# AnishDelft/ModelCompression

Measured on AMD Instinct MI355X. Metric: images/sec (fwd+bwd, 416x416), higher is better.
Workload: dtype fp16

## Files before the change

include/mcamd.h:

```cpp
#ifndef MCAMD_H
#define MCAMD_H

#include <stddef.h>
#include <stdint.h>

#ifdef __cplusplus
extern "C" {
#endif

#define MCAMD_OK 0
#define MCAMD_EINVAL (-1)
#define MCAMD_ELAUNCH (-2)
#define MCAMD_EWORKSPACE (-3)

int mcamd_version(void);
void mcamd_reload_config(void);
const char* mcamd_arch(void);
const char* mcamd_last_error(void);

typedef struct mcamd_conv_geom {
    int32_t B, H, W;
    int32_t ksize;
    int32_t cin;
    int32_t cout;
// ... 164 lines not shown
    int32_t ch_lo, C;
} mcamd_dgrad_sums;
int32_t mcamd_conv_dgrad_sums_rows(const mcamd_conv_geom* g, int32_t concurrent);
int mcamd_conv_dgrad_sums(const mcamd_conv_geom* g, const void* dy, int32_t dy_ld, int32_t dy_choff,
                          const void* wp_dgrad, const mcamd_conv_epilogue* epi, const mcamd_dgrad_sums* sums, void* stream);

size_t mcamd_conv_wgrad_workspace_bytes(const mcamd_conv_geom* g);
int mcamd_conv_wgrad(const mcamd_conv_geom* g, const void* x, const void* dy, int32_t dy_ld,
                     int32_t dy_choff, const float* mask_oihw, const mcamd_chan_map* map,
                     float grad_scale, float* dw_oihw, float* dbias, void* workspace,
                     size_t workspace_bytes, void* stream);

#define MCAMD_WGRAD_GENERIC 0
#define MCAMD_WGRAD_STEM 1
#define MCAMD_WGRAD_WIN 2
#define MCAMD_WGRAD_NINE 3
#define MCAMD_WGRAD_NINE_WIDE 4
#define MCAMD_WFIN_ROW 0
#define MCAMD_WFIN_VEC 1
#define MCAMD_WFIN_GENERIC 2
#define MCAMD_WGRAD_PLAN_INFO_N 13
int mcamd_conv_wgrad_plan_info(const mcamd_conv_geom* g, int32_t has_cmap, int32_t out[MCAMD_WGRAD_PLAN_INFO_N]);
int32_t mcamd_wgrad_generic_instances(int32_t* out, int32_t cap);

int mcamd_bn_coeffs(const float* stats, int32_t stats_rows, int32_t stats_ld, int32_t C, int64_t count,
                    const float* gamma, const float* beta, float* running_mean, float* running_var,
                    float momentum, float eps, int32_t training,
                    float* scale, float* shift, float* save_mean, float* save_invstd,
                    const int32_t* chan_perm, void* stream);

int mcamd_bn_coeffs_ex(const float* stats, int32_t stats_rows, int32_t stats_ld, int32_t C, int64_t count,
                       const float* gamma, const float* beta, float* running_mean, float* running_var,
                       float momentum, float eps, int32_t training,
                       float* scale, float* shift, float* save_mean, float* save_invstd,
                       const int32_t* chan_perm, int32_t ones_channel, void* stream);

#define MCAMD_DST_PLAIN 0
#define MCAMD_DST_POOL 1
#define MCAMD_DST_REORG 2
typedef struct mcamd_act_desc {
    int32_t B, H, W, C;
    const void* y; int32_t y_ld, y_choff;
    const float* scale; const float* shift;
    float slope;
    int32_t mode;
    void* dst; int32_t dst_ld, dst_choff;
// ... 353 lines not shown
```

modelcompression_amd/_lib.py:

```python
import ctypes as C
import os

_HERE = os.path.dirname(os.path.abspath(__file__))
LIB_PATH = os.path.join(_HERE, "libmcamd.so")


class McamdError(RuntimeError):
    pass


class ConvGeom(C.Structure):
    _fields_ = [("B", C.c_int32), ("H", C.c_int32), ("W", C.c_int32), ("ksize", C.c_int32),
                ("cin", C.c_int32), ("cout", C.c_int32), ("x_ld", C.c_int32), ("x_choff", C.c_int32),
                ("stem", C.c_int32), ("pad", C.c_int32), ("x_wrap", C.c_int32), ("x_f8", C.c_int32), ("x_f8_wexp", C.c_int32)]


class ConvEpilogue(C.Structure):
    _fields_ = [("mode", C.c_int32), ("y_ld", C.c_int32), ("y_choff", C.c_int32),
                ("y", C.c_void_p), ("bias", C.c_void_p), ("stats", C.c_void_p),
                ("stats_rows", C.c_int32), ("stats_ld", C.c_int32),
                ("scale", C.c_void_p), ("shift", C.c_void_p), ("slope", C.c_float), ("overflow", C.c_void_p),
                ("dst_mode", C.c_int32), ("y2", C.c_void_p), ("y2_ld", C.c_int32), ("y2_choff", C.c_int32),
                ("concurrent", C.c_int32)]

# ... 215 lines not shown
    "mcamd_conv_fwd_q8_sparse24_ok": (_I32, [C.POINTER(ConvGeom)]),
    "mcamd_q8_sparse24_elems": (C.c_int, [C.POINTER(ConvGeom), C.POINTER(_I64)]),
    "mcamd_pack_q8_sparse24": (C.c_int, [C.POINTER(ConvGeom), _P, _P, _P, _P, _P, _P]),
    "mcamd_conv_fwd_q8_sparse24": (C.c_int, [C.POINTER(ConvGeom), _P, _P, _P, _P, C.POINTER(ConvEpilogue), _I32, _I32, _P]),
    "mcamd_conv_fwd_q8_w4_ok": (_I32, [C.POINTER(ConvGeom)]),
    "mcamd_q8_w4_elems": (C.c_int, [C.POINTER(ConvGeom), C.POINTER(_I64)]),
    "mcamd_pack_q8_w4": (C.c_int, [C.POINTER(ConvGeom), _P, _P, _P, _P, _P, _P]),
    "mcamd_unpack_q8_w4": (C.c_int, [C.POINTER(ConvGeom), _P, _P, _P, _P]),
    "mcamd_conv_fwd_q8_w4": (C.c_int, [C.POINTER(ConvGeom), _P, _P, _P, _P, C.POINTER(ConvEpilogue), _I32, _I32, _P]),
    "mcamd_conv_fwd_q8_w4_info": (C.c_int, [C.POINTER(ConvGeom), C.POINTER(_I32)]),
    "mcamd_conv_fwd_q8_w4_raw": (C.c_int, [C.POINTER(ConvGeom), _P, _P, _P, _P, C.POINTER(ConvEpilogue), _P]),
    "mcamd_fakequant_q8_w4": (C.c_int, [C.POINTER(ConvGeom), _P, _P, _P, _P, _P]),
    "mcamd_cast_q8": (C.c_int, [_P, _I64, _I32, _I32, _I32, _P, _I32, _I32, _P]),
    "mcamd_conv_fwd_q8_stats_rows": (_I32, [C.POINTER(ConvGeom)]),
    "mcamd_fakequant_q8": (C.c_int, [C.POINTER(ConvGeom), _P, _P, _P, _P, _P]),
    "mcamd_cast_q8_train": (C.c_int, [_P, _I64, _I32, _I32, _I32, _P, _I32, _I32, _P]),
    "mcamd_conv_dgrad": (C.c_int, [C.POINTER(ConvGeom), _P, _I32, _I32, _P, C.POINTER(ConvEpilogue), _P]),
    "mcamd_conv_dgrad_sums_rows": (_I32, [C.POINTER(ConvGeom), _I32]),
    "mcamd_conv_dgrad_sums": (C.c_int, [C.POINTER(ConvGeom), _P, _I32, _I32, _P, C.POINTER(ConvEpilogue), C.POINTER(DgradSums), _P]),
    "mcamd_conv_wgrad_workspace_bytes": (_SZ, [C.POINTER(ConvGeom)]),
    "mcamd_conv_wgrad": (C.c_int, [C.POINTER(ConvGeom), _P, _P, _I32, _I32, _P, C.POINTER(ChanMap), _F, _P, _P, _P, _SZ, _P]),
    "mcamd_conv_wgrad_plan_info": (C.c_int, [C.POINTER(ConvGeom), _I32, C.POINTER(_I32)]),
    "mcamd_wgrad_generic_instances": (_I32, [C.POINTER(_I32), _I32]),
    "mcamd_bn_coeffs": (C.c_int, [_P, _I32, _I32, _I32, _I64, _P, _P, _P, _P, _F, _F, _I32, _P, _P, _P, _P, _P, _P]),
    "mcamd_bn_coeffs_ex": (C.c_int, [_P, _I32, _I32, _I32, _I64, _P, _P, _P, _P, _F, _F, _I32, _P, _P, _P, _P, _P, _I32, _P]),
    "mcamd_fold_weights": (C.c_int, [C.POINTER(FoldDesc), _P, _P]),
    "mcamd_fold_weights_many": (C.c_int, [_P, _I32, _I64, _P]),
    "mcamd_unfold_wgrad": (C.c_int, [C.POINTER(FoldDesc), _P, _P, _P, _P, _I32, _P]),
    "mcamd_bn_act_fwd": (C.c_int, [C.POINTER(ActDesc), _P]),
    "mcamd_bn_act_fwd_instance": (C.c_int, [C.POINTER(ActDesc), C.POINTER(ActInstance)]),
    "mcamd_bn_act_conv1x1_ok": (_I32, [C.POINTER(ActDesc), C.POINTER(ConvGeom)]),
    "mcamd_bn_act_conv1x1_stats_rows": (_I32, [C.POINTER(ActDesc), C.POINTER(ConvGeom)]),
    "mcamd_bn_act_conv1x1_info": (C.c_int, [C.POINTER(ActDesc), C.POINTER(ConvGeom), C.POINTER(BnConv1x1Instance)]),
    "mcamd_bn_act_conv1x1_fwd": (C.c_int, [C.POINTER(ActDesc), C.POINTER(ConvGeom), _P, C.POINTER(ConvEpilogue), _P]),
    "mcamd_bn_act_bwd_workspace_bytes": (_SZ, [C.POINTER(ActBwdDesc)]),
    "mcamd_bn_act_bwd": (C.c_int, [C.POINTER(ActBwdDesc), _P, _SZ, _P]),
    "mcamd_stem_block_workspace_bytes": (_SZ, []),
    "mcamd_stem_block_fwd": (C.c_int, [C.POINTER(StemBlockDesc), _P, _SZ, _P]),
    "mcamd_stem_block_bwd": (C.c_int, [C.POINTER(StemBlockDesc), _P, _SZ, _P]),
    "mcamd_stem_block_stats_rows": (_I32, [C.POINTER(StemBlockDesc)]),
    "mcamd_stem_block_stats": (C.c_int, [C.POINTER(StemBlockDesc), _P, _I32, _I32, _P]),
    "mcamd_stem_block_plan_info": (C.c_int, [C.POINTER(StemBlockDesc), C.POINTER(_I32)]),
    "mcamd_nchw_f32_to_nhwc4_split": (C.c_int, [_P, _I32, _I32, _I32, _P, _P, _P]),
    "mcamd_pack_stem_split": (C.c_int, [_P, _P, _I32, _P, _P, _P]),
    "mcamd_nchw_f32_to_padded_nhwc_f16": (C.c_int, [_P, _I32, _I32, _I32, _I32, _F, _P, _I32, _I32, _P, _P]),
    "mcamd_nchw_f32_to_padded_nhwc_f16_pad": (C.c_int, [_P, _I32, _I32, _I32, _I32, _F, _P, _I32, _I32, _I32, _P, _P]),
# ... 94 lines not shown
```

modelcompression_amd/build.py:

```python
import os
import subprocess
import sys
from concurrent.futures import ThreadPoolExecutor

HERE = os.path.dirname(os.path.abspath(__file__))
CSRC = os.path.join(HERE, "csrc")
OUT = os.path.join(HERE, "libmcamd.so")
HIPCC = os.environ.get("HIPCC", "/opt/rocm/bin/hipcc")
ARCH = "gfx950"
COMMON = ["--offload-arch=" + ARCH, "-O3", "-fPIC", "-std=c++17", "-Wall", "-Wno-unused-variable",
          "-fhip-fp32-correctly-rounded-divide-sqrt"]
SOURCES = {
    "api.hip": [],
    "conv_igemm.hip": [],
    "conv_igemm_pp.hip": [],
    "conv_sparse.hip": [],
    "conv_bsparse.hip": [],
    "conv_splitk.hip": [],
    "conv_q8.hip": [],
    "conv_q8_sparse.hip": [],
    "conv_q8_splitk.hip": [],
    "conv_q8_bsparse.hip": [],
    "conv_q8_w4.hip": [],
    "conv_stem.hip": [],
    "conv_stem_block.hip": [],
    "conv_stem_f32.hip": [],
    "conv_small.hip": [],
    "conv_win.hip": [],
    "conv_wres.hip": [],
    "conv_wgrad.hip": [],
    "conv_wgrad_stem.hip": [],
    "bn_act.hip": [],
    "bn_conv1x1.hip": [],
    "fold.hip": [],
    "plan.hip": [],
    "region_loss.hip": [],
    "distill_loss.hip": [],
    "prune.hip": ["-ffp-contract=off"],
    "augment.hip": ["-ffp-contract=off"],
    "detect.hip": ["-ffp-contract=off"],
    "voc_eval.hip": ["-ffp-contract=off"],
    "wpack.hip": ["-ffp-contract=off"],
    "wshare.hip": ["-ffp-contract=off"],
    "huff.hip": [],
    "taylor.hip": ["-ffp-contract=off"],
}


def _stale(target, deps):
    if not os.path.exists(target):
        return True
    t = os.path.getmtime(target)
    return any(os.path.getmtime(d) > t for d in deps)

# ... 34 lines not shown
```

modelcompression_amd/csrc/api.hip:

```cpp
#include <stdarg.h>
#include <stdlib.h>
#include <string.h>

#include <string>

#include "kernels.h"

static thread_local char g_err[512] = "";

void mcamd_set_error(const char* fmt, ...) {
    va_list ap;
    va_start(ap, fmt);
    vsnprintf(g_err, sizeof(g_err), fmt, ap);
    va_end(ap);
}

int g_mcamd_env_generation = 0;
int McamdEnvSlot::get(const char* name, int dflt) {
    const int g = __atomic_load_n(&g_mcamd_env_generation, __ATOMIC_ACQUIRE);
    if (gen != g) {
        const char* s = getenv(name);
        has = s && *s ? 1 : 0;
        val = has ? atoi(s) : 0;
        __atomic_store_n(&gen, g, __ATOMIC_RELEASE);
// ... 1312 lines not shown
    a.dy_off = dy_choff + a.dy_row_stride + dy_ld;
    a.dy_zero_off = dy_choff;
    a.H = g->H, a.W = g->W, a.HW = g->H * g->W;
    a.M = (int)M;
    a.cin_tap = cin_tap;
    a.ntaps = ntaps;
    a.ktot = ntaps * cin_tap;
    fill_taps(g->ksize, g->stem, a.x_row_stride, g->x_ld, a.tap_off);
    int rc = p.nine    ? mcamd_wgrad9_launch(a, p, g->W + pw_of(g), padded_pixels(g), st)
             : p.stemw == 1 ? mcamd_wgrad_stem_launch(a, p, st)
             : p.stemw == 2 ? mcamd_wgrad_win_launch(a, p, st)
                       : mcamd_wgrad_launch(a, p, st);
    if (rc) return rc;
    rc = mcamd_wgrad_finish_launch((const float*)workspace, p, a.ktot, cin_tap, g->stem, g->cout, g->cin, g->ksize,
                                   mask_oihw, 1.0f / grad_scale, dw_oihw, rmap, cmap, st);
    if (rc) return rc;
    if (dbias) {
        long long rows = padded_pixels(g);
        rc = mcamd_colsum_launch((const half_t*)dy, rows, dy_ld, dy_choff, g->cout, 1.0f / grad_scale, dbias, st, workspace,
                                 workspace_bytes);
    }
    return rc;
}
```

modelcompression_amd/csrc/kernels.h:

```cpp
#pragma once
#include "common.h"

struct DgradSums {
    float* slab;
    const half_t* act;
    const float* scale;
    const float* shift;
    const float* mean;
    const float* invstd;
    const float* y;
    int act_ld, act_choff, act_pw;
    int y_ld, y_choff;
    int ch_lo, C;
    int ld;
    float slope;
};
#define MCAMD_EPI_RAW_F16_SUMS 4

struct IgemmArgs {
    const half_t* x;
    const half_t* w;
    void* y;
    const float* bias;
    float* stats;
// ... 134 lines not shown
int mcamd_conv_q8_w4_raw_launch(IgemmArgs& a, const void* gshift, const void* wexp, hipStream_t st);
int mcamd_fakequant_q8_w4_launch(const void* codes, const void* gshift, const void* wexp, float* out, int cout, int cin, int ntaps,
                                 hipStream_t st);

WgradPlan mcamd_wgrad_plan(long long M, int cout, int cin_tap, int ntaps);
int mcamd_wgrad_launch(WgradArgs& a, const WgradPlan& p, hipStream_t st);
bool mcamd_wgrad_stem_ok(int stem, int cout, int W, long long M);
WgradPlan mcamd_wgrad_stem_plan(long long M);
int mcamd_wgrad_stem_launch(WgradArgs& a, const WgradPlan& p, hipStream_t st);
bool mcamd_wgrad_win_ok(int ksize, int stem, int cout, int cin_tap, int W, long long M);
WgradPlan mcamd_wgrad_win_plan(long long M, int cout);
int mcamd_wgrad_win_launch(WgradArgs& a, const WgradPlan& p, hipStream_t st);
bool mcamd_wgrad_use9(int ksize, int stem, int cout, int cin_tap, int W);
WgradPlan mcamd_wgrad_plan9(long long P, int cout, int cin_tap, int W, int pitch, int B);
int mcamd_wgrad9_launch(const WgradArgs& w, const WgradPlan& p, int pitch, long long P, hipStream_t st);
WgradFinish mcamd_wgrad_finish_pick(int nsplit, int stem, int Cin, int ksize, bool has_cmap);
int mcamd_wgrad_instances(int (*out)[4], int cap);
int mcamd_wgrad_finish_launch(const float* slab, const WgradPlan& p, int ktot, int cin_tap, int stem, int Cout, int Cin,
                              int ksize, const float* mask, float inv_scale, float* dw, const int* rmap, const int* cmap,
                              hipStream_t st);
int mcamd_colsum_launch(const half_t* dy, long long rows, int ld, int choff, int C, float inv_scale, float* out,
                        hipStream_t st, void* scratch, size_t scratch_bytes);

bool mcamd_win3x3_ok(int mode, bool stats, long long M, int n, int cin_tap, int ktot, int H, int W);
int mcamd_win3x3_launch(const IgemmArgs& a, hipStream_t st);
bool mcamd_small3x3_ok(long long M, int n, int cin_tap, int ktot);
int mcamd_small3x3_rows(long long M);
int mcamd_small3x3_launch(const IgemmArgs& a, int rows, hipStream_t st);
bool mcamd_small3x3_split_ok(long long M, int n, int cin_tap, int ktot, int wrap, int mode);
int mcamd_small3x3_split_launch(const IgemmArgs& a, int rows, hipStream_t st);

bool mcamd_bn_conv1x1_shape_ok(int P, int cout);
struct BnConv1x1Choice { int bn, cb, threads, rows, num_mtiles, grid, lds_bytes; };
bool mcamd_bn_conv1x1_choice(int P, int cout, long long M, int rows, BnConv1x1Choice* c);
int mcamd_bn_conv1x1_launch(IgemmArgs& a, const float* py, int py_ld, int py_choff, int P, int rows, hipStream_t st);

bool mcamd_wres_ok(int ksize, int stem, int n, int cin_tap, int ktot, int B, int H, int W, int mode);
int mcamd_wres_rows(int n, int B, int H, int W);
int mcamd_wres_launch(IgemmArgs& a, int B, int rows, hipStream_t st);

bool mcamd_stem_direct_ok(int stem, int cout, int mode);
int mcamd_stem_rows(long long M);
int mcamd_stem_launch(const StemArgs& a, int cout, int rows, hipStream_t st);
```

modelcompression_amd/engine.py:

```python
import contextlib
import math
import os
import time

import torch

from . import ops
from . import _lib as L
from ._lib import McamdError


class _T:
    __slots__ = ("buf", "ld", "choff", "C", "H", "W", "ps", "ps0")

    def __init__(self, buf, ld, choff, C, H, W, ps=0):
        self.buf, self.ld, self.choff, self.C, self.H, self.W, self.ps = buf, ld, choff, C, H, W, ps
        self.ps0 = ps


_LAYER_FIELDS = dict(
    index=0, li=0, conv=None, bn=None, slope=1.0, src=0, tin=None, cin=0, cout=0, cout_p=0, H=0, W=0, k=0, M=0, stem=0, pad=0,
    level=1, mode=0, out_id=None, out2_id=None, out_t=None, out2_t=None, is_last=False, train_ok=True, border=None,
    border_map=None, geom=None, geom_f=None, p_lo=0, p_hi=0,
    wp=None, wd=None, y=None, stats=None, scale=None, shift=None, mean=None, invstd=None, dy=None, gin=None, act_full=None,
# ... 309 lines not shown
        self.overlap_wgrad = os.environ.get("MCAMD_OVERLAP_WGRAD", "1") == "1"
        self.wgrad_chunk = 1
        self.use_plan = os.environ.get("MCAMD_PLAN", "1") == "1"
        self._fwd_plans, self._bwd_plan, self._plan_epoch = {}, None, 0
        self._logits = self._gout = self._flat = None
        self._pack_on_side = False
        self.sparse_layers = []
        self.bsparse_layers = []
        self.bsparse_kept = {}
        self._bs_exempt = frozenset()
        self.splitk_layers = []
        self._splitk_ws = None
        self._form_key = (None, None, None, None, None)
        self._training, self._fold_key = None, None
        self.fold_dead = os.environ.get("MCAMD_FOLD_DEAD", "1") == "1"
        self.f8 = precision == "mixed" and os.environ.get("MCAMD_F8", "1") == "1"
        self.bn_narrow_on = True
        self.bwd_from_act = True
        self.pool_act_on = True
        self.dgrad_bn_sums = os.environ.get("MCAMD_DGRAD_BN_SUMS", "1") == "1"
        self.fuse_bn_1x1 = os.environ.get("MCAMD_FUSE_BN_1X1", "1") == "1"
        self.fused_1x1_launches = 0
        self._fused_1x1_cache = {}
        self._dgrad_sums_cache = {}
        self._side_stream = None
        self._side_concurrent = True
        self._side_ws = None
        self.overflow = torch.zeros(1, dtype=torch.int32, device=device)
        self._build_plan(H, W)

    def _build_plan(self, H0, W0):
        model, B, dev = self.model, self.B, self.device
        blocks = model.blocks
        bops = _resolve_routes(blocks)
        n = len(bops)

        def alias(t):
            while t >= 0 and bops[t][0] == "route" and len(bops[t][1]) == 1:
                t = bops[t][1][0]
            return t

        srcs = [[alias(s) for s in o[1]] for o in bops]
        consumers = {}
        for ind, (t, _) in enumerate(bops):
            if t == "route" and len(srcs[ind]) == 1:
                continue
# ... 1048 lines not shown
        if lay.xq is not None:
            ti, x8 = lay.tin, lay.xq
            self._timed('cast', lay, ops.cast_q8, xin, ops.padded_pixels(B, ti.H, ti.W, self._pad_for(ti.W)), ti.ld, ti.choff,
                        lay.cin, x8, ti.ld, ti.choff, write_back=True)
        _FORMS[lay.form].qat_raw(self, lay, x8)
        ops.bn_coeffs(lay.stats, lay.cout, lay.M, bn.weight.data, bn.bias.data, bn.running_mean, bn.running_var, True,
                      lay.scale, lay.shift, lay.mean, lay.invstd, momentum=_momentum(bn), eps=bn.eps)
        t, t2 = lay.out_t, lay.out2_t
        dst2, dst2_pad = self._dst2(t2)
        ops.bn_act_fwd(B, lay.H, lay.W, lay.cout, lay.y, lay.cout, 0, lay.scale, lay.shift, lay.slope, lay.mode,
                       self.bufs[t.buf], t.ld, t.choff, *dst2, dst_pad=self._pad_for(t.W), dst2_pad=dst2_pad,
                       dst_q8=self.qbufs[t.buf] if lay.q8_y else None,
                       dst2_q8=self.qbufs[t2.buf] if (t2 is not None and lay.q8_y2) else None)

    def _stem_split_forward(self, lay):
        bn, t = lay.bn, lay.out_t
        ops.stem_block_stats(self.B, lay.H, lay.W, lay.sh_img, lay.sh_wp, lay.stats, x_lo=lay.sh_img_lo, wp_lo=lay.sh_wp_lo)
        ops.bn_coeffs(lay.stats, lay.cout, lay.M, bn.weight.data, bn.bias.data, bn.running_mean, bn.running_var, True,
                      lay.scale, lay.shift, lay.mean, lay.invstd, momentum=_momentum(bn), eps=bn.eps)
        ops.stem_block_fwd(self.B, lay.H, lay.W, lay.sh_img, lay.sh_wp, bn.weight.data, bn.bias.data, None, None, False,
                           lay.scale, lay.shift, lay.mean, lay.invstd, lay.slope, self.bufs[t.buf], t.ld, t.choff, None,
                           eps=bn.eps, cout=lay.cout, planes=self.act_planes, x_lo=lay.sh_img_lo, wp_lo=lay.sh_wp_lo)

    def _dgrad_sums(self, lay, concurrent):
        if not (self.dgrad_bn_sums and self.bwd_from_act and self.precise) or lay.gin is None:
            return None
        key = (lay.li, bool(concurrent), self._plan_epoch)
        hit = self._dgrad_sums_cache.get(key, False)
        if hit is not False:
            return hit
        res = None
        if lay.fold is None and not lay.gather and lay.in_perm is None and lay.geom_act is lay.geom:
            for prod in self.layers:
                if prod.is_last or prod.fused_stem or prod.stem_shadow or prod.bn is None or prod.out_t is None:
                    continue
                if self.consumer_of.get(prod.out_id) is not lay or prod.mode != L.DST_PLAIN or prod.slope <= 0.0:
                    continue
                if prod.out2_id is not None and prod.out2_id in self.consumer_of:
                    continue
                if (prod.keep is not None or prod.perm is not None or prod.fold is not None or prod.skip_dead or prod.fold_consumers
                        or prod.bn_width or prod.border is not None or prod.cout % 8 != 0):
                    continue
                t = prod.out_t
                ch_lo = t.choff - lay.tin.choff
                if t.buf != lay.tin.buf or t.ld != lay.tin.ld or ch_lo < 0 or ch_lo % 8 != 0 or ch_lo + prod.cout > lay.geom.cin:
                    continue
                rows = ops.dgrad_sums_rows(lay.geom_act, concurrent)
                if rows <= 0:
                    continue
                slab = torch.empty(rows, 2, prod.cout, dtype=torch.float32, device=self.device)
                y = prod.y if (prod.y is not None and prod.y.dtype == torch.float32) else None
                desc = ops.dgrad_sums(slab, self.bufs[t.buf], t.ld, t.choff, self._pad_for(t.W), prod.scale, prod.shift, prod.mean,
                                      prod.invstd, prod.slope, prod.cout, ch_lo=ch_lo, y=y, y_ld=prod.cout, y_choff=0)
                res = (desc, slab, prod)
                break
        self._dgrad_sums_cache = {k: v for k, v in self._dgrad_sums_cache.items() if k[2] == self._plan_epoch}
        self._dgrad_sums_cache[key] = res
        return res

    def bn_act_bwd_layer(self, lay, g, g_ld, g_choff, g2, g2_ld, g2_choff, dy, dgamma, dbeta, grad_scale, sums=None):
        cb = lay.bn_width or lay.cout
        act = {}
        if self.bwd_from_act and self.precise and lay.mode == L.DST_PLAIN and g2 is None:
            t = lay.out_t
            act = dict(act=self.bufs[t.buf], act_ld=t.ld, act_choff=t.choff, act_pad=self._pad_for(t.W))
        elif self.bwd_from_act and self.precise and self.train_layout and lay.mode == L.DST_POOL and lay.slope > 0.0:
            if self.pool_act_on and lay.act_full is not None:
                act = dict(act=lay.act_full, act_ld=ops.round_up(lay.cout, 8), act_choff=0, act_pad=self._pad_for(lay.W))
            if g2 is None and lay.y is not None:
                t = lay.out_t
# ... 22 lines not shown
        side = None
        if self.overlap_wgrad and self.events is None:
            side = self._get_side_stream()
            if self._side_ws is None or self._side_ws.numel() < self.wgrad_ws.numel():
                self._side_ws = torch.empty(self.wgrad_ws.numel(), dtype=torch.uint8, device=self.device)
                self._side_ws.record_stream(side)
                self._plan_epoch += 1

        def fence():
            ev2 = torch.cuda.Event()
            ev2.record(main)
            side.wait_event(ev2)
            return torch.cuda.stream(side)

        def on_side():
            return torch.cuda.stream(side)

        def ready(lay):
            if on_ready is None:
                return
            if side is None:
                on_ready(flat, lay.p_lo, lay.p_hi)
            elif getattr(on_ready, "takes_fence", False):
                on_ready(flat, lay.p_lo, lay.p_hi, fence if (lay.fused_stem or lay.stem_shadow) else on_side)
            else:
                with fence():
                    on_ready(flat, lay.p_lo, lay.p_hi)

        if self.use_plan and self.events is None:
            key = (main.cuda_stream, side.cuda_stream if side is not None else 0, D, self._plan_epoch, self._ptr_sig())
            plan = self._bwd_plan
            if plan is None or plan.key != key:
                plan = ops.Plan([main] + ([side] if side is not None else []))
                seg_lays = [[]]

                def close_segment(lay):
                    seg_lays[-1].append(lay)
                    plan.mark()
                    seg_lays.append([])
                with plan:
                    self._backward_body(gmap, main, side, S, D, close_segment)
                plan.key, plan.seg_lays = key, seg_lays
                self._bwd_plan = plan
            if on_ready is None:
                plan.run()
            else:
                for si in range(plan.segments):
# ... 34 lines not shown
            if lay.fused_stem:
                flush()
                cons = self.consumer_of[lay.out_id]
                mask = lay.conv.mask.contiguous() if lay.conv.mask_flag else None
                self._timed('wgrad', lay, ops.stem_block_bwd, self.B, lay.H, lay.W, self.bufs[lay.tin.buf], lay.wp,
                            lay.bn.weight.data, lay.scale, lay.shift, lay.mean, lay.invstd, lay.slope, cons.gin, cons.tin.ld,
                            lay.out_t.choff, gmap[id(lay.conv.weight)], gmap[id(lay.bn.weight)], gmap[id(lay.bn.bias)],
                            lay.stem_ws, mask=mask, grad_scale=D)
                ready(lay)
                continue
            if lay.is_last:
                ops.nchw_to_padded(self._gout, lay.dy, lay.cout_p, 0, S, overflow=self.overflow, pad=lay.pad)
            else:
                cons = self.consumer_of[lay.out_id]
                t = lay.out_t
                g2 = g2_ld = g2_choff = None
                if lay.out2_id is not None and lay.out2_id in self.consumer_of:
                    c2, t2 = self.consumer_of[lay.out2_id], lay.out2_t
                    g2, g2_ld, g2_choff = c2.gin, c2.tin.ld, t2.choff
                self.bn_act_bwd_layer(lay, cons.gin, cons.tin.ld, t.choff, g2, g2_ld or 0, g2_choff or 0, lay.dy,
                                      gmap[id(lay.bn.weight)], gmap[id(lay.bn.bias)], D, sums=sums_of.pop(lay.li, None))
            mask = lay.conv.mask.contiguous() if lay.conv.mask_flag else None
            dbias = gmap[id(lay.conv.bias)] if lay.conv.bias is not None else None
            def wgrad_of(ws, lay=lay, mask=mask, dbias=dbias):
                if lay.fold is not None:
                    gw, prod = gmap[id(lay.conv.weight)], lay.fold
                    if lay.perm is not None:
                        ops.memset_zero(gw)
                    self._timed('wgrad', lay, ops.conv_wgrad, lay.geom_act, self.bufs[lay.tin.buf], lay.dy, lay.cout_p, 0,
                                lay.dwaug, None, D, dbias, ws)
                    ops.unfold_wgrad(lay.conv.weight.data, mask, lay.g_rows, lay.g_cols, prod.bn.bias.data, prod.slope, lay.n_act,
                                     lay.fold_cin, lay.dwaug, gw, gmap[id(prod.bn.bias)], gmap[id(prod.bn.weight)],
                                     accumulate=prod.fold_consumers[0] is not lay)
                elif lay.gather:
                    gw = gmap[id(lay.conv.weight)]
                    if lay.perm is not None:
                        ops.memset_zero(gw)
                    self._timed('wgrad', lay, ops.conv_wgrad, lay.geom_act, self.bufs[lay.tin.buf], lay.dy, lay.cout_p, 0,
                                gw, mask, D, dbias, ws, rows=lay.g_rows, cols=lay.g_cols)
                else:
                    self._timed('wgrad', lay, ops.conv_wgrad, lay.geom, self.bufs[lay.tin.buf], lay.dy, lay.cout_p, 0,
                                gmap[id(lay.conv.weight)], mask, D, dbias, ws)

            if side is None:
                wgrad_of(self.wgrad_ws)
                ready(lay)
# ... 15 lines not shown
```

modelcompression_amd/ops.py:

```python
import collections
import ctypes as C
import weakref

import torch

from . import _lib as L
from ._lib import (ConvGeom, ConvEpilogue, SplitkInfo, ActDesc, ActBwdDesc, DgradSums, ChanMap, PackJob, StemBlockDesc, FoldDesc, FoldJob, check, ptr,
                   stream_ptr)

HALF = torch.float16
SLACK = 64


def round_up(v, m):
    return (v + m - 1) // m * m


def _need_cuda(*ts):
    for t in ts:
        if t is not None and not t.is_cuda:
            raise L.McamdError("modelcompression_amd compute ops need CUDA (MI355X) tensors; there is no CPU path")


def guard_elems(W, ld):
# ... 205 lines not shown

WgradPlanInfo = collections.namedtuple("WgradPlanInfo", "family tmo tnc taps kp ns nsplit pix_per_split rows_pad finish sg tiles grid")


def wgrad_plan_info(g, has_cmap=False):
    out = (C.c_int32 * L.WGRAD_PLAN_INFO_N)()
    check(L.lib().mcamd_conv_wgrad_plan_info(C.byref(g), 1 if has_cmap else 0, out), "mcamd_conv_wgrad_plan_info")
    return WgradPlanInfo(*out)


def wgrad_generic_instances():
    lib = L.lib()
    n = int(lib.mcamd_wgrad_generic_instances(None, 0))
    out = (C.c_int32 * (4 * n))()
    lib.mcamd_wgrad_generic_instances(out, n)
    return [tuple(out[4 * i:4 * i + 4]) for i in range(n)]


def conv_wgrad(g, x, dy, dy_ld, dy_choff, dw, mask=None, grad_scale=1.0, dbias=None, workspace=None, rows=None, cols=None):
    if workspace is None:
        workspace = torch.empty(wgrad_workspace_bytes(g), dtype=torch.uint8, device=dw.device)
    check(L.lib().mcamd_conv_wgrad(C.byref(g), ptr(x), ptr(dy), dy_ld, dy_choff, ptr(mask), _chan_map(g, rows, cols), grad_scale, ptr(dw),
                                   ptr(dbias), ptr(workspace), workspace.numel(), stream_ptr()), "mcamd_conv_wgrad")


def _perm_ptr(perm, C_):
    if perm is None:
        return None
    if perm.dtype != torch.int32 or perm.numel() != C_ or not perm.is_contiguous() or not perm.is_cuda:
        raise L.McamdError("channel permutation must be a contiguous CUDA int32 vector of %d entries" % C_)
    return perm.data_ptr()


def bn_coeffs(stats, C_, count, gamma, beta, rmean, rvar, training, scale, shift, mean=None, invstd=None,
              momentum=0.1, eps=1e-5, perm=None, ones_channel=-1):
    rows = stats.shape[0] if stats is not None else 0
    ld = stats.shape[2] if stats is not None else 0
    check(L.lib().mcamd_bn_coeffs_ex(ptr(stats), rows, ld, C_, count, ptr(gamma), ptr(beta), ptr(rmean), ptr(rvar),
                                     momentum, eps, 1 if training else 0, ptr(scale), ptr(shift), ptr(mean), ptr(invstd),
                                     _perm_ptr(perm, C_), ones_channel, stream_ptr()), "mcamd_bn_coeffs_ex")


def _fold_desc(w, mask, rows, cols, beta, slope, n, cin_k, aug):
    _need_cuda(w, mask, rows, cols, beta)
    assert w.dtype == torch.float32 and w.is_contiguous() and w.dim() == 4 and w.shape[2] == w.shape[3]
    assert beta.dtype == torch.float32 and beta.numel() == w.shape[1]
# ... 1327 lines not shown
```

Baseline: 5693.

## Fuse 1x1 conv dgrad and wgrad into one backward kernel sharing tiles

Adds a fused backward kernel for 1x1 convolutions. Each dY tile is loaded into LDS once and used for both the input gradient (MFMA against the weights) and the weight gradient partials, which go into a per-block slab. The kernel can also accumulate the producer's batch-norm backward sums from the same tile. The engine routes eligible layers to it by default, in place of separate dgrad and wgrad launches, and runs them on the main stream instead of the side stream. This cuts reading dY and x twice and the launch overhead, at the cost of losing dgrad/wgrad concurrency and adding a slab reduction plus a fixed 256-block grid.

```diff
diff --git a/include/mcamd.h b/include/mcamd.h
--- a/include/mcamd.h
+++ b/include/mcamd.h
@@ -210,6 +210,15 @@
 #define MCAMD_WGRAD_PLAN_INFO_N 13
 int mcamd_conv_wgrad_plan_info(const mcamd_conv_geom* g, int32_t has_cmap, int32_t out[MCAMD_WGRAD_PLAN_INFO_N]);
 int32_t mcamd_wgrad_generic_instances(int32_t* out, int32_t cap);
+
+int32_t mcamd_conv_bwd1x1_ok(const mcamd_conv_geom* g, const char** reason);
+int32_t mcamd_conv_bwd1x1_sums_rows(const mcamd_conv_geom* g);
+int32_t mcamd_conv_bwd1x1_wgrad_splits(const mcamd_conv_geom* g);
+size_t mcamd_conv_bwd1x1_workspace_bytes(const mcamd_conv_geom* g);
+int mcamd_conv_bwd1x1(const mcamd_conv_geom* g, const void* x, const void* dy, int32_t dy_ld, int32_t dy_choff,
+                      const void* wp_dgrad, void* gin, int32_t g_ld, int32_t g_choff, int32_t* overflow,
+                      const mcamd_dgrad_sums* sums, const float* mask_oihw, float grad_scale, float* dw_oihw, float* dbias,
+                      void* workspace, size_t workspace_bytes, void* stream);
 
 int mcamd_bn_coeffs(const float* stats, int32_t stats_rows, int32_t stats_ld, int32_t C, int64_t count,
                     const float* gamma, const float* beta, float* running_mean, float* running_var,
diff --git a/modelcompression_amd/_lib.py b/modelcompression_amd/_lib.py
--- a/modelcompression_amd/_lib.py
+++ b/modelcompression_amd/_lib.py
@@ -261,6 +261,12 @@
     "mcamd_conv_wgrad": (C.c_int, [C.POINTER(ConvGeom), _P, _P, _I32, _I32, _P, C.POINTER(ChanMap), _F, _P, _P, _P, _SZ, _P]),
     "mcamd_conv_wgrad_plan_info": (C.c_int, [C.POINTER(ConvGeom), _I32, C.POINTER(_I32)]),
     "mcamd_wgrad_generic_instances": (_I32, [C.POINTER(_I32), _I32]),
+    "mcamd_conv_bwd1x1_ok": (_I32, [C.POINTER(ConvGeom), C.POINTER(C.c_char_p)]),
+    "mcamd_conv_bwd1x1_sums_rows": (_I32, [C.POINTER(ConvGeom)]),
+    "mcamd_conv_bwd1x1_wgrad_splits": (_I32, [C.POINTER(ConvGeom)]),
+    "mcamd_conv_bwd1x1_workspace_bytes": (_SZ, [C.POINTER(ConvGeom)]),
+    "mcamd_conv_bwd1x1": (C.c_int, [C.POINTER(ConvGeom), _P, _P, _I32, _I32, _P, _P, _I32, _I32, _P, C.POINTER(DgradSums), _P, _F,
+                                    _P, _P, _P, _SZ, _P]),
     "mcamd_bn_coeffs": (C.c_int, [_P, _I32, _I32, _I32, _I64, _P, _P, _P, _P, _F, _F, _I32, _P, _P, _P, _P, _P, _P]),
     "mcamd_bn_coeffs_ex": (C.c_int, [_P, _I32, _I32, _I32, _I64, _P, _P, _P, _P, _F, _F, _I32, _P, _P, _P, _P, _P, _I32, _P]),
     "mcamd_fold_weights": (C.c_int, [C.POINTER(FoldDesc), _P, _P]),
diff --git a/modelcompression_amd/build.py b/modelcompression_amd/build.py
--- a/modelcompression_amd/build.py
+++ b/modelcompression_amd/build.py
@@ -30,6 +30,7 @@
     "conv_wres.hip": [],
     "conv_wgrad.hip": [],
     "conv_wgrad_stem.hip": [],
+    "conv_bwd1x1.hip": [],
     "bn_act.hip": [],
     "bn_conv1x1.hip": [],
     "fold.hip": [],
diff --git a/modelcompression_amd/csrc/api.hip b/modelcompression_amd/csrc/api.hip
--- a/modelcompression_amd/csrc/api.hip
+++ b/modelcompression_amd/csrc/api.hip
@@ -1358,3 +1358,95 @@
     }
     return rc;
 }
+
+static const char* bwd1x1_refusal(const mcamd_conv_geom* g) {
+    if (!g) return "null geometry";
+    if (g->pad != 0 && g->pad != 1) return "pad must be 0 or 1";
+    const char* why = mcamd_bwd1x1_refusal(g->ksize, g->stem, g->x_wrap, g->x_f8, g->cout, g->cin);
+    if (why) return why;
+    if (g->x_ld % 8 != 0 || g->x_choff % 8 != 0 || g->x_choff < 0 || g->x_choff + g->cin > g->x_ld)
+        return "x channel slice must be whole groups of 8 inside x_ld";
+    if (g->B <= 0 || g->H <= 0 || g->W <= 0 || (long long)g->B * g->H * g->W >= (1ll << 31)) return "pixel count out of range";
+    return nullptr;
+}
+
+extern "C" int32_t mcamd_conv_bwd1x1_ok(const mcamd_conv_geom* g, const char** reason) {
+    const char* why = bwd1x1_refusal(g);
+    if (reason) *reason = why;
+    return why ? 0 : 1;
+}
+
+extern "C" int32_t mcamd_conv_bwd1x1_sums_rows(const mcamd_conv_geom* g) { return bwd1x1_refusal(g) ? 0 : MCAMD_BWD1X1_GRID; }
+extern "C" int32_t mcamd_conv_bwd1x1_wgrad_splits(const mcamd_conv_geom* g) { return bwd1x1_refusal(g) ? 0 : MCAMD_BWD1X1_GRID; }
+extern "C" size_t mcamd_conv_bwd1x1_workspace_bytes(const mcamd_conv_geom* g) {
+    return bwd1x1_refusal(g) ? 0 : (size_t)MCAMD_BWD1X1_GRID * g->cout * g->cin * sizeof(float);
+}
+
+extern "C" int mcamd_conv_bwd1x1(const mcamd_conv_geom* g, const void* x, const void* dy, int32_t dy_ld, int32_t dy_choff,
+                                 const void* wp_dgrad, void* gin, int32_t g_ld, int32_t g_choff, int32_t* overflow,
+                                 const mcamd_dgrad_sums* sums, const float* mask_oihw, float grad_scale, float* dw_oihw,
+                                 float* dbias, void* workspace, size_t workspace_bytes, void* stream) {
+    if (mcamd_recording()) {
+        MCAMD_REQUIRE(g, "conv_bwd1x1: null geometry");
+        const mcamd_conv_geom g_ = *g;
+        const bool has_sums = sums != nullptr;
+        const mcamd_dgrad_sums s_ = has_sums ? *sums : mcamd_dgrad_sums{};
+        return mcamd_rec_push(stream, [=](void* s) {
+            return mcamd_conv_bwd1x1(&g_, x, dy, dy_ld, dy_choff, wp_dgrad, gin, g_ld, g_choff, overflow, has_sums ? &s_ : nullptr,
+                                     mask_oihw, grad_scale, dw_oihw, dbias, workspace, workspace_bytes, s);
+        });
+    }
+    const char* why = bwd1x1_refusal(g);
+    MCAMD_REQUIRE(!why, "conv_bwd1x1: %s", why);
+    MCAMD_REQUIRE(x && dy && wp_dgrad && gin && dw_oihw && workspace, "conv_bwd1x1: null argument");
+    MCAMD_REQUIRE(grad_scale > 0.f, "conv_bwd1x1: grad_scale must be positive");
+    MCAMD_REQUIRE(dy_ld % 8 == 0 && dy_choff % 8 == 0 && dy_choff >= 0 && dy_choff + g->cout <= dy_ld,
+                  "conv_bwd1x1: dy slice [%d, %d) does not fit dy_ld %d", dy_choff, dy_choff + g->cout, dy_ld);
+    MCAMD_REQUIRE(g_ld % 8 == 0 && g_choff % 8 == 0 && g_choff >= 0 && g_choff + g->cin <= g_ld,
+                  "conv_bwd1x1: G slice [%d, %d) does not fit g_ld %d", g_choff, g_choff + g->cin, g_ld);
+    const size_t need = mcamd_conv_bwd1x1_workspace_bytes(g);
+    if (workspace_bytes < need) {
+        mcamd_set_error("conv_bwd1x1: workspace %zu < %zu bytes", workspace_bytes, need);
+        return MCAMD_EWORKSPACE;
+    }
+    Bwd1x1Launch q;
+    memset(&q, 0, sizeof(q));
+    q.dy = (const half_t*)dy, q.x = (const half_t*)x, q.w = (const half_t*)wp_dgrad, q.g = (half_t*)gin;
+    q.slab = (float*)workspace, q.overflow = (int*)overflow;
+    q.dy_ld = dy_ld, q.dy_choff = dy_choff, q.x_ld = g->x_ld, q.x_choff = g->x_choff, q.g_ld = g_ld, q.g_choff = g_choff;
+    q.H = g->H, q.W = g->W, q.M = g->B * g->H * g->W, q.pw = pw_of(g), q.cout = g->cout, q.cin = g->cin;
+    if (sums && sums->slab) {
+        const mcamd_dgrad_sums* s = sums;
+        MCAMD_REQUIRE(s->rows == MCAMD_BWD1X1_GRID, "conv_bwd1x1: sums.rows must be mcamd_conv_bwd1x1_sums_rows() = %d (got %d)",
+                      MCAMD_BWD1X1_GRID, s->rows);
+        MCAMD_REQUIRE(s->scale && s->shift && s->mean && s->invstd, "conv_bwd1x1: sums: null argument");
+        MCAMD_REQUIRE(s->C > 0 && s->C % 8 == 0 && s->ch_lo >= 0 && s->ch_lo % 8 == 0 && s->ch_lo + s->C <= g->cin,
+                      "conv_bwd1x1: sums: producer columns [%d, %d) must be whole groups of 8 inside the %d channels of G",
+                      s->ch_lo, s->ch_lo + s->C, g->cin);
+        MCAMD_REQUIRE(s->ld >= s->C, "conv_bwd1x1: sums.ld (%d) must be >= C (%d)", s->ld, s->C);
+        MCAMD_REQUIRE(s->act == x && s->act_ld == g->x_ld && s->act_choff == g->x_choff + s->ch_lo && (s->act_pad != 0) == (g->pad != 0),
+                      "conv_bwd1x1: sums: the producer's activation must be the block's input x (same buffer, ld, form; act_choff = "
+                      "x_choff + ch_lo)");
+        MCAMD_REQUIRE(!s->y || (s->y_ld % 4 == 0 && s->y_choff % 4 == 0 && s->y_choff >= 0 && s->y_choff + s->C <= s->y_ld),
+                      "conv_bwd1x1: sums: fp32 y slice [%d, %d) does not fit y_ld %d", s->y_choff, s->y_choff + s->C, s->y_ld);
+        MCAMD_REQUIRE(s->slope > 0.f, "conv_bwd1x1: sums need an invertible activation (slope > 0)");
+        q.bsum.slab = s->slab, q.bsum.ld = s->ld;
+        q.bsum.scale = s->scale, q.bsum.shift = s->shift, q.bsum.mean = s->mean, q.bsum.invstd = s->invstd;
+        q.bsum.y = s->y, q.bsum.y_ld = s->y_ld, q.bsum.y_choff = s->y_choff;
+        q.bsum.ch_lo = s->ch_lo, q.bsum.C = s->C;
+        q.bsum.slope = s->slope;
+    }
+    hipStream_t st = (hipStream_t)stream;
+    int rc = mcamd_bwd1x1_launch(q, st);
+    if (rc) return rc;
+    WgradPlan p;
+    memset(&p, 0, sizeof(p));
+    p.nsplit = MCAMD_BWD1X1_GRID, p.rows_pad = g->cout;
+    rc = mcamd_wgrad_finish_launch((const float*)workspace, p, g->cin, g->cin, 0, g->cout, g->cin, 1, mask_oihw, 1.0f / grad_scale,
+                                   dw_oihw, nullptr, nullptr, st);
+    if (rc) return rc;
+    if (dbias)
+        rc = mcamd_colsum_launch((const half_t*)dy, padded_pixels(g), dy_ld, dy_choff, g->cout, 1.0f / grad_scale, dbias, st, workspace,
+                                 workspace_bytes);
+    return rc;
+}
diff --git a/modelcompression_amd/csrc/conv_bwd1x1.hip b/modelcompression_amd/csrc/conv_bwd1x1.hip
--- /dev/null
+++ b/modelcompression_amd/csrc/conv_bwd1x1.hip
@@ -0,0 +1,306 @@
+#include "conv_epi.h"
+#include "tr_frag.h"
+#include <string.h>
+
+struct Bwd1x1Args {
+    const half_t* dy;
+    const half_t* x;
+    const half_t* w;
+    half_t* g;
+    float* slab;
+    int* overflow;
+    int dy_ld, dy_choff, x_ld, x_choff, g_ld, g_choff;
+    int H, W, HW, M, pw;
+    int ntiles;
+    DgradSums bsum;
+};
+
+__device__ __forceinline__ void step_pixel(int b0, int h0, int w0, int r, int H, int W, int& b, int& h, int& w) {
+    b = b0, h = h0, w = w0 + r;
+    while (w >= W) w -= W, ++h;
+    while (h >= H) h -= H, ++b;
+}
+
+template <int COUT, int CIN, int P>
+__global__ __launch_bounds__(512, 1) void bwd1x1_kernel(Bwd1x1Args a) {
+    constexpr int NT = 512;
+    constexpr int A_CH = COUT / 8, B_CH = CIN / 8;
+    constexpr int A_IT = P * A_CH / NT, B_IT = P * B_CH / NT;
+    constexpr int A_RS = NT / A_CH, B_RS = NT / B_CH;
+    constexpr int RBA = COUT * 2;
+    constexpr int NH = CIN / 128;
+    constexpr int XPLANE = P * 256;
+    constexpr int GP = CIN + 4;
+    constexpr int SA = 0, SX = P * RBA, SG = SX + NH * XPLANE, SW = SG + P * GP * 2;
+    constexpr int KS = COUT / 16;
+    constexpr int NCB = CIN / 32;
+    constexpr int PBW = (P / 32) / (8 / NCB);
+    constexpr int DI = COUT / 64, DJ = CIN / 128;
+    static_assert(RBA == 256 || RBA == 128, "dY rows of 64 or 128 filters");
+    static_assert(CIN % 128 == 0 && NCB <= 8 && PBW >= 1 && A_IT >= 1 && B_IT >= 1, "tile shape");
+    static_assert(P * A_CH % NT == 0 && P * B_CH % NT == 0 && NT % B_CH == 0 && CIN * A_CH % NT == 0, "whole pieces per thread");
+
+    extern __shared__ __attribute__((aligned(16))) char smem[];
+    const int tid = threadIdx.x, lane = tid & 63;
+    const int wave = __builtin_amdgcn_readfirstlane(tid >> 6);
+
+    const int t0 = (int)((long long)blockIdx.x * a.ntiles / gridDim.x);
+    const int t1 = (int)((long long)(blockIdx.x + 1) * a.ntiles / gridDim.x);
+
+    const int cb = wave % NCB, pb0 = (wave / NCB) * PBW;
+#pragma unroll
+    for (int it = 0; it < CIN * A_CH / NT; ++it) {
+        const int piece = it * NT + tid, c = piece / A_CH, ch = piece % A_CH;
+        *(h8_t*)(smem + SW + c * RBA + ((ch ^ (c & (A_CH - 1))) << 4)) = *(const h8_t*)(a.w + c * COUT + ch * 8);
+    }
+    const int wrow = cb * 32 + (lane & 31);
+    const char* wlane = smem + SW + wrow * RBA;
+
+    const bool SUMS = a.bsum.slab != nullptr;
+    const int sch = tid % B_CH, srow0 = tid / B_CH;
+    const int sc0 = sch * 8 - a.bsum.ch_lo;
+    const bool live = SUMS && sc0 >= 0 && sc0 < a.bsum.C;
+    float sb[8], sg[8], off[8], mul[8];
+    bool usey[8];
+    bool need_y = false;
+#pragma unroll
+    for (int i = 0; i < 8; ++i) sb[i] = sg[i] = 0.f, off[i] = 0.f, mul[i] = 0.f, usey[i] = false;
+    if (live) {
+        float sc[8], sh[8], mu[8], is[8];
+#pragma unroll
+        for (int i = 0; i < 8; ++i)
+            sc[i] = a.bsum.scale[sc0 + i], sh[i] = a.bsum.shift[sc0 + i], mu[i] = a.bsum.mean[sc0 + i], is[i] = a.bsum.invstd[sc0 + i];
+        need_y = act_xhat_source(sc, sh, mu, is, a.bsum.y != nullptr, off, mul, usey);
+#pragma unroll
+        for (int i = 0; i < 8; ++i) mul[i] = usey[i] ? 0.f : mul[i];
+    }
+    const float slope = a.bsum.slope, inv_slope = SUMS ? 1.0f / slope : 1.f;
+
+    f32x16_t dw[DI][DJ];
+#pragma unroll
+    for (int i = 0; i < DI; ++i)
+#pragma unroll
+        for (int j = 0; j < DJ; ++j)
+#pragma unroll
+            for (int r = 0; r < 16; ++r) dw[i][j][r] = 0.f;
+    bool sat = false;
+
+    h8_t ra[A_IT], rb[B_IT];
+    auto load_tile = [&](int t) {
+        const int m0 = t * P;
+        int b0, h0, w0;
+        split_pixel(m0, a.HW, a.W, b0, h0, w0);
+#pragma unroll
+        for (int it = 0; it < A_IT; ++it) {
+            const int row = tid / A_CH + it * A_RS, ch = tid % A_CH;
+            int b, h, w;
+            step_pixel(b0, h0, w0, m0 + row < a.M ? row : a.M - 1 - m0, a.H, a.W, b, h, w);
+            ra[it] = *(const h8_t*)(a.dy + pad_off(b, h, w, a.H, a.W, a.dy_ld, a.pw) + a.dy_choff + ch * 8);
+        }
+#pragma unroll
+        for (int it = 0; it < B_IT; ++it) {
+            const int row = tid / B_CH + it * B_RS, ch = tid % B_CH;
+            int b, h, w;
+            step_pixel(b0, h0, w0, m0 + row < a.M ? row : a.M - 1 - m0, a.H, a.W, b, h, w);
+            rb[it] = *(const h8_t*)(a.x + pad_off(b, h, w, a.H, a.W, a.x_ld, a.pw) + a.x_choff + ch * 8);
+        }
+    };
+    auto put_tile = [&](int t) {
+        const int mlim = a.M - t * P;
+        const h8_t zero = {0, 0, 0, 0, 0, 0, 0, 0};
+#pragma unroll
+        for (int it = 0; it < A_IT; ++it) {
+            const int row = tid / A_CH + it * A_RS, ch = tid % A_CH;
+            *(h8_t*)(smem + SA + row * RBA + ((ch ^ tr_swz<RBA>(row)) << 4)) = row < mlim ? ra[it] : zero;
+        }
+#pragma unroll
+        for (int it = 0; it < B_IT; ++it) {
+            const int row = tid / B_CH + it * B_RS, ch = tid % B_CH;
+            *(h8_t*)(smem + SX + (ch >> 4) * XPLANE + row * 256 + (((ch & 15) ^ tr_swz<256>(row)) << 4)) = row < mlim ? rb[it] : zero;
+        }
+    };
+
+    if (t0 < t1) load_tile(t0);
+    for (int t = t0; t < t1; ++t) {
+        put_tile(t);
+        __syncthreads();
+        if (t + 1 < t1) load_tile(t + 1);
+
+        {
+            f32x16_t g[PBW];
+#pragma unroll
+            for (int q = 0; q < PBW; ++q)
+#pragma unroll
+                for (int r = 0; r < 16; ++r) g[q][r] = 0.f;
+#pragma unroll
+            for (int s = 0; s < KS; ++s) {
+                const h8_t wfs = *(const h8_t*)(wlane + (((2 * s + (lane >> 5)) ^ (wrow & (A_CH - 1))) << 4));
+#pragma unroll
+                for (int q = 0; q < PBW; ++q) {
+                    const int row = (pb0 + q) * 32 + (lane & 31), ch = 2 * s + (lane >> 5);
+                    const h8_t df = *(const h8_t*)(smem + SA + row * RBA + ((ch ^ tr_swz<RBA>(row)) << 4));
+                    g[q] = __builtin_amdgcn_mfma_f32_32x32x16_f16(wfs, df, g[q], 0, 0, 0);
+                }
+            }
+            half_t* gt = (half_t*)(smem + SG);
+#pragma unroll
+            for (int q = 0; q < PBW; ++q) {
+                const int row = (pb0 + q) * 32 + (lane & 31);
+#pragma unroll
+                for (int v = 0; v < 4; ++v) {
+                    h4_t hv;
+#pragma unroll
+                    for (int e = 0; e < 4; ++e) {
+                        const float f = g[q][4 * v + e];
+                        sat |= fabsf(f) > 65504.f;
+                        hv[e] = (half_t)fminf(fmaxf(f, -65504.f), 65504.f);
+                    }
+                    *(h4_t*)(gt + row * GP + cb * 32 + 8 * v + 4 * (lane >> 5)) = hv;
+                }
+            }
+        }
+        __syncthreads();
+
+        {
+            const half_t* gt = (const half_t*)(smem + SG);
+#pragma unroll
+            for (int k = 0; k < B_IT; ++k) {
+                const int row = srow0 + k * B_RS, m = t * P + row;
+                if (m >= a.M) continue;
+                const h4_t g0 = *(const h4_t*)(gt + row * GP + sch * 8), g1 = *(const h4_t*)(gt + row * GP + sch * 8 + 4);
+                const h8_t gq = __builtin_shufflevector(g0, g1, 0, 1, 2, 3, 4, 5, 6, 7);
+                *(h8_t*)(a.g + (long long)m * a.g_ld + a.g_choff + sch * 8) = gq;
+                if (!live) continue;
+                const h8_t av8 = *(const h8_t*)(smem + SX + (sch >> 4) * XPLANE + row * 256 + (((sch & 15) ^ tr_swz<256>(row)) << 4));
+                float z[8];
+#pragma unroll
+                for (int i = 0; i < 8; ++i) {
+                    const float av = (float)av8[i];
+                    z[i] = av > 0.f ? av : av * inv_slope;
+                }
+#pragma unroll
+                for (int i = 0; i < 8; ++i) {
+                    const float gv = (float)gq[i];
+                    const float gz = (float)av8[i] > 0.f ? gv : gv * slope;
+                    sb[i] += gz;
+                    sg[i] += gz * ((z[i] - off[i]) * mul[i]);
+                }
+            }
+        }
+
+#pragma unroll
+        for (int s = 0; s < P / 16; ++s) {
+            h8_t af[DI], bf[DJ];
+#pragma unroll
+            for (int i = 0; i < DI; ++i) af[i] = tr_frag_rows_builtin<RBA>(smem + SA, 16 * s, ((wave >> 2) * DI + i) * 32, lane);
+#pragma unroll
+            for (int j = 0; j < DJ; ++j) {
+                const int col = ((wave & 3) * DJ + j) * 32;
+                bf[j] = tr_frag_rows_builtin<256>(smem + SX + (col >> 7) * XPLANE, 16 * s, col & 127, lane);
+            }
+#pragma unroll
+            for (int i = 0; i < DI; ++i)
+#pragma unroll
+                for (int j = 0; j < DJ; ++j) dw[i][j] = __builtin_amdgcn_mfma_f32_32x32x16_f16(af[i], bf[j], dw[i][j], 0, 0, 0);
+        }
+        __syncthreads();
+    }
+
+    if (need_y) {
+        float sc[8], sh[8], mu[8], is[8], off2[8], mul2[8];
+#pragma unroll
+        for (int i = 0; i < 8; ++i)
+            sc[i] = a.bsum.scale[sc0 + i], sh[i] = a.bsum.shift[sc0 + i], mu[i] = a.bsum.mean[sc0 + i], is[i] = a.bsum.invstd[sc0 + i];
+        act_xhat_source(sc, sh, mu, is, true, off2, mul2, usey);
+        for (int t = t0; t < t1; ++t)
+            for (int k = 0; k < B_IT; ++k) {
+                const int m = t * P + srow0 + k * B_RS;
+                if (m >= a.M) continue;
+                int b, h, w;
+                split_pixel(m, a.HW, a.W, b, h, w);
+                const h8_t gq = *(const h8_t*)(a.g + (long long)m * a.g_ld + a.g_choff + sch * 8);
+                const h8_t av8 = *(const h8_t*)(a.x + pad_off(b, h, w, a.H, a.W, a.x_ld, a.pw) + a.x_choff + sch * 8);
+                const float* yp = a.bsum.y + (long long)m * a.bsum.y_ld + a.bsum.y_choff + sc0;
+#pragma unroll
+                for (int i = 0; i < 8; ++i) {
+                    const float gv = (float)gq[i];
+                    const float gz = (float)av8[i] > 0.f ? gv : gv * slope;
+                    if (usey[i]) sg[i] += gz * ((yp[i] - off2[i]) * mul2[i]);
+                }
+            }
+    }
+
+    if (sat && a.overflow) atomicOr(a.overflow, 1);
+
+    float* out = a.slab + (long long)blockIdx.x * COUT * CIN;
+#pragma unroll
+    for (int i = 0; i < DI; ++i)
+#pragma unroll
+        for (int j = 0; j < DJ; ++j)
+#pragma unroll
+            for (int r = 0; r < 16; ++r) {
+                const int n = ((wave >> 2) * DI + i) * 32 + mfma32_row(r, lane);
+                const int k = ((wave & 3) * DJ + j) * 32 + (lane & 31);
+                out[n * CIN + k] = dw[i][j][r];
+            }
+
+    if (SUMS) {
+        constexpr int PITCH = NT + 8;
+        float* red = (float*)smem;
+#pragma unroll
+        for (int i = 0; i < 8; ++i) {
+            red[i * PITCH + tid] = sb[i];
+            red[(8 + i) * PITCH + tid] = sg[i];
+        }
+        __syncthreads();
+        for (int e = tid; e < 2 * CIN; e += NT) {
+            const int which = e / CIN, col = e - which * CIN;
+            const int c = col - a.bsum.ch_lo;
+            if (c < 0 || c >= a.bsum.C) continue;
+            const int v = which * 8 + (col & 7), chq = col >> 3;
+            float s = 0.f;
+            for (int r = 0; r < B_RS; ++r) s += red[v * PITCH + r * B_CH + chq];
+            a.bsum.slab[((long long)blockIdx.x * 2 + which) * a.bsum.ld + c] = s;
+        }
+    }
+}
+
+#define BWD1X1_INSTANCES(X) X(64, 128, 128) X(128, 256, 64)
+
+const char* mcamd_bwd1x1_refusal(int ksize, int stem, int x_wrap, int x_f8, int cout, int cin) {
+    if (ksize != 1) return "ksize must be 1";
+    if (stem || x_wrap != 0 || x_f8 != 0) return "dense geometry only (no stem / x_wrap / x_f8 form)";
+    if (cout % 8 != 0 || cin % 8 != 0) return "cout and cin must be multiples of 8";
+#define B_OK(CO_, CI_, P_) \
+    if (cout == CO_ && cin == CI_) return nullptr;
+    BWD1X1_INSTANCES(B_OK)
+#undef B_OK
+    return "no kernel instance for this (cout, cin): (64, 128) and (128, 256) exist";
+}
+
+int mcamd_bwd1x1_launch(const Bwd1x1Launch& q, hipStream_t st) {
+    Bwd1x1Args a;
+    memset(&a, 0, sizeof(a));
+    a.dy = q.dy, a.x = q.x, a.w = q.w, a.g = q.g, a.slab = q.slab, a.overflow = q.overflow;
+    a.dy_ld = q.dy_ld, a.dy_choff = q.dy_choff, a.x_ld = q.x_ld, a.x_choff = q.x_choff, a.g_ld = q.g_ld, a.g_choff = q.g_choff;
+    a.H = q.H, a.W = q.W, a.HW = q.H * q.W, a.M = q.M, a.pw = q.pw;
+    a.bsum = q.bsum;
+    bool done = false;
+#define B_CASE(CO_, CI_, P_)                                                                        \
+    if (!done && q.cout == CO_ && q.cin == CI_) {                                                   \
+        constexpr size_t lds = (size_t)P_ * CO_ * 2 + (size_t)P_ * CI_ * 2 + (size_t)P_ * (CI_ + 4) * 2 + (size_t)CO_ * CI_ * 2; \
+        static_assert(lds >= 16 * (512 + 8) * sizeof(float), "the sums reduction reuses the tiles");  \
+        a.ntiles = (q.M + P_ - 1) / P_;                                                             \
+        MCAMD_LDS_OPT_IN((bwd1x1_kernel<CO_, CI_, P_>), lds);                                       \
+        hipLaunchKernelGGL((bwd1x1_kernel<CO_, CI_, P_>), dim3(MCAMD_BWD1X1_GRID), dim3(512), lds, st, a); \
+        done = true;                                                                                \
+    }
+    BWD1X1_INSTANCES(B_CASE)
+#undef B_CASE
+    if (!done) {
+        mcamd_set_error("conv_bwd1x1: no kernel instance for cout %d cin %d", q.cout, q.cin);
+        return MCAMD_EINVAL;
+    }
+    MCAMD_LAUNCH_CHECK("conv_bwd1x1");
+    return MCAMD_OK;
+}
diff --git a/modelcompression_amd/csrc/kernels.h b/modelcompression_amd/csrc/kernels.h
--- a/modelcompression_amd/csrc/kernels.h
+++ b/modelcompression_amd/csrc/kernels.h
@@ -180,6 +180,21 @@
 int mcamd_colsum_launch(const half_t* dy, long long rows, int ld, int choff, int C, float inv_scale, float* out,
                         hipStream_t st, void* scratch, size_t scratch_bytes);
 
+#define MCAMD_BWD1X1_GRID 256
+struct Bwd1x1Launch {
+    const half_t* dy;
+    const half_t* x;
+    const half_t* w;
+    half_t* g;
+    float* slab;
+    int* overflow;
+    int dy_ld, dy_choff, x_ld, x_choff, g_ld, g_choff;
+    int H, W, M, pw, cout, cin;
+    DgradSums bsum;
+};
+const char* mcamd_bwd1x1_refusal(int ksize, int stem, int x_wrap, int x_f8, int cout, int cin);
+int mcamd_bwd1x1_launch(const Bwd1x1Launch& q, hipStream_t st);
+
 bool mcamd_win3x3_ok(int mode, bool stats, long long M, int n, int cin_tap, int ktot, int H, int W);
 int mcamd_win3x3_launch(const IgemmArgs& a, hipStream_t st);
 bool mcamd_small3x3_ok(long long M, int n, int cin_tap, int ktot);
diff --git a/modelcompression_amd/engine.py b/modelcompression_amd/engine.py
--- a/modelcompression_amd/engine.py
+++ b/modelcompression_amd/engine.py
@@ -355,6 +355,9 @@
         self.fuse_bn_1x1 = os.environ.get("MCAMD_FUSE_BN_1X1", "1") == "1"
         self.fused_1x1_launches = 0
         self._fused_1x1_cache = {}
+        self.bwd1x1 = os.environ.get("MCAMD_BWD1X1", "1") == "1"
+        self._bwd1x1_cache = {}
+        self._bwd1x1_ws = None
         self._dgrad_sums_cache = {}
         self._side_stream = None
         self._side_concurrent = True
@@ -1449,10 +1452,25 @@
                            lay.scale, lay.shift, lay.mean, lay.invstd, lay.slope, self.bufs[t.buf], t.ld, t.choff, None,
                            eps=bn.eps, cout=lay.cout, planes=self.act_planes, x_lo=lay.sh_img_lo, wp_lo=lay.sh_wp_lo)
 
-    def _dgrad_sums(self, lay, concurrent):
+    def _bwd1x1_route(self, lay):
+        if not self.bwd1x1 or lay.li == 0 or lay.gin is None or lay.fused_stem or lay.stem_shadow:
+            return False
+        key = (lay.li, self._plan_epoch)
+        hit = self._bwd1x1_cache.get(key)
+        if hit is None:
+            hit = (lay.fold is None and not lay.gather and lay.in_perm is None and lay.geom_act is lay.geom
+                   and ops.conv_bwd1x1_ok(lay.geom)[0])
+            self._bwd1x1_cache = {k: v for k, v in self._bwd1x1_cache.items() if k[1] == self._plan_epoch}
+            self._bwd1x1_cache[key] = hit
+        if hit and self._bwd1x1_ws is None:
+            need = max(ops.conv_bwd1x1_workspace_bytes(l.geom) for l in self.layers if l.geom is not None)
+            self._bwd1x1_ws = torch.empty(need, dtype=torch.uint8, device=self.device)
+        return hit
+
+    def _dgrad_sums(self, lay, concurrent, fused=False):
         if not (self.dgrad_bn_sums and self.bwd_from_act and self.precise) or lay.gin is None:
             return None
-        key = (lay.li, bool(concurrent), self._plan_epoch)
+        key = (lay.li, "fused" if fused else bool(concurrent), self._plan_epoch)
         hit = self._dgrad_sums_cache.get(key, False)
         if hit is not False:
             return hit
@@ -1472,7 +1490,7 @@
                 ch_lo = t.choff - lay.tin.choff
                 if t.buf != lay.tin.buf or t.ld != lay.tin.ld or ch_lo < 0 or ch_lo % 8 != 0 or ch_lo + prod.cout > lay.geom.cin:
                     continue
-                rows = ops.dgrad_sums_rows(lay.geom_act, concurrent)
+                rows = ops.conv_bwd1x1_sums_rows(lay.geom) if fused else ops.dgrad_sums_rows(lay.geom_act, concurrent)
                 if rows <= 0:
                     continue
                 slab = torch.empty(rows, 2, prod.cout, dtype=torch.float32, device=self.device)
@@ -1541,7 +1559,8 @@
             if side is None:
                 on_ready(flat, lay.p_lo, lay.p_hi)
             elif getattr(on_ready, "takes_fence", False):
-                on_ready(flat, lay.p_lo, lay.p_hi, fence if (lay.fused_stem or lay.stem_shadow) else on_side)
+                on_ready(flat, lay.p_lo, lay.p_hi,
+                         fence if (lay.fused_stem or lay.stem_shadow or self._bwd1x1_route(lay)) else on_side)
             else:
                 with fence():
                     on_ready(flat, lay.p_lo, lay.p_hi)
@@ -1622,6 +1641,16 @@
                                       gmap[id(lay.bn.weight)], gmap[id(lay.bn.bias)], D, sums=sums_of.pop(lay.li, None))
             mask = lay.conv.mask.contiguous() if lay.conv.mask_flag else None
             dbias = gmap[id(lay.conv.bias)] if lay.conv.bias is not None else None
+            if self._bwd1x1_route(lay):
+                flush()
+                ds = self._dgrad_sums(lay, False, fused=True)
+                if ds is not None:
+                    sums_of[ds[2].li] = ds[1]
+                self._timed('dgrad', lay, ops.conv_bwd1x1, lay.geom, self.bufs[lay.tin.buf], lay.dy, lay.cout_p, 0, lay.wd,
+                            lay.gin, lay.tin.ld, lay.tin.choff, gmap[id(lay.conv.weight)], mask=mask, grad_scale=D, dbias=dbias,
+                            workspace=self._bwd1x1_ws, overflow=self.overflow, sums=ds[0] if ds is not None else None)
+                ready(lay)
+                continue
             def wgrad_of(ws, lay=lay, mask=mask, dbias=dbias):
                 if lay.fold is not None:
                     gw, prod = gmap[id(lay.conv.weight)], lay.fold
diff --git a/modelcompression_amd/ops.py b/modelcompression_amd/ops.py
--- a/modelcompression_amd/ops.py
+++ b/modelcompression_amd/ops.py
@@ -251,6 +251,33 @@
         workspace = torch.empty(wgrad_workspace_bytes(g), dtype=torch.uint8, device=dw.device)
     check(L.lib().mcamd_conv_wgrad(C.byref(g), ptr(x), ptr(dy), dy_ld, dy_choff, ptr(mask), _chan_map(g, rows, cols), grad_scale, ptr(dw),
                                    ptr(dbias), ptr(workspace), workspace.numel(), stream_ptr()), "mcamd_conv_wgrad")
+
+
+def conv_bwd1x1_ok(g):
+    why = C.c_char_p()
+    ok = bool(L.lib().mcamd_conv_bwd1x1_ok(C.byref(g), C.byref(why)))
+    return ok, (None if ok else why.value.decode())
+
+
+def conv_bwd1x1_sums_rows(g):
+    return int(L.lib().mcamd_conv_bwd1x1_sums_rows(C.byref(g)))
+
+
+def conv_bwd1x1_wgrad_splits(g):
+    return int(L.lib().mcamd_conv_bwd1x1_wgrad_splits(C.byref(g)))
+
+
+def conv_bwd1x1_workspace_bytes(g):
+    return int(L.lib().mcamd_conv_bwd1x1_workspace_bytes(C.byref(g)))
+
+
+def conv_bwd1x1(g, x, dy, dy_ld, dy_choff, wpd, gin, g_ld, g_choff, dw, mask=None, grad_scale=1.0, dbias=None, workspace=None,
+                overflow=None, sums=None):
+    if workspace is None:
+        workspace = torch.empty(conv_bwd1x1_workspace_bytes(g), dtype=torch.uint8, device=dw.device)
+    check(L.lib().mcamd_conv_bwd1x1(C.byref(g), ptr(x), ptr(dy), dy_ld, dy_choff, ptr(wpd), ptr(gin), g_ld, g_choff, ptr(overflow),
+                                    C.byref(sums) if sums is not None else None, ptr(mask), grad_scale, ptr(dw), ptr(dbias),
+                                    ptr(workspace), workspace.numel(), stream_ptr()), "mcamd_conv_bwd1x1")
 
 
 def _perm_ptr(perm, C_):
```

Measured after the change: 5759 (median of 6 runs). +1.2%, better.
